# julius-speech/julius

Hardware: NVIDIA H100
Metric: frames/sec (xRT) 20k-word triphone decode (higher is better)
Workload: dtype f32

## Files before the change

### julius_b200/csrc/common.cuh

```cuda
#pragma once
#include <cuda_runtime.h>
#include <cstdint>
#include <cstdio>
#include <cstring>
#include <string>
#include <atomic>
#include <vector>
#include "julius_b200.h"

namespace jb200 {

void set_error(const char *fmt, ...);
extern std::atomic<int64_t> g_launches;

static constexpr int ADDLOG_TABLE_N = 500000;
void build_addlog_table(std::vector<float> &tbl);
__device__ __forceinline__ float addlog_step_exact(float y, float x, const float *__restrict__ tbl) {
  if (x > y) { float t = x; x = y; y = t; }
  float tmp = __fsub_rn(x, y);
  if (tmp < __double2float_ru(JB200_LOG_ADDMIN)) return y;
  unsigned int idx = (unsigned int)__dadd_rn(__dmul_rn((double)(-tmp), 33333.3333), 0.5);
  return __fadd_rn(y, __ldg(tbl + idx));
}

struct SpliceSeg { int row0, frame0, carry0, n_carry, n_win; };
struct SpliceMap {
  const SpliceSeg *seg = nullptr;
  int nseg = 0;
  const float *carry = nullptr;
};
__device__ __forceinline__ const float *splice_frame(const SpliceSeg &s, int k, const float *in, const float *carry, int fl) {
  return (k < s.n_carry) ? carry + (size_t)(s.carry0 + k) * fl : in + (size_t)(s.frame0 + k - s.n_carry) * fl;
}

#define JB_CUDA(expr)                                                              \
  do {                                                                             \
    cudaError_t _e = (expr);                                                       \
    if (_e != cudaSuccess) {                                                       \
      jb200::set_error("%s failed: %s (%s:%d)", #expr, cudaGetErrorString(_e), __FILE__, __LINE__); \
      return JB200_ERR_CUDA;                                                       \
    }                                                                              \
  } while (0)

#define JB_RC(expr)                                                                \
  do {                                                                             \
    const int _rc = (expr);                                                        \
    if (_rc != JB200_OK) return _rc;                                               \
  } while (0)

#define JB_LAUNCH_CHECK()                                                          \
  do {                                                                             \
    jb200::g_launches.fetch_add(1, std::memory_order_relaxed);                     \
    cudaError_t _e = cudaGetLastError();                                           \
    if (_e != cudaSuccess) {                                                       \
      jb200::set_error("kernel launch failed: %s (%s:%d)", cudaGetErrorString(_e), __FILE__, __LINE__); \
      return JB200_ERR_CUDA;                                                       \
    }                                                                              \
  } while (0)

__device__ __forceinline__ uint32_t smem_u32(const void *p) {
  return static_cast<uint32_t>(__cvta_generic_to_shared(p));
}
__device__ __forceinline__ void mbar_init(uint64_t *bar, uint32_t count) {
  asm volatile("mbarrier.init.shared::cta.b64 [%0], %1;" ::"r"(smem_u32(bar)), "r"(count));
}
__device__ __forceinline__ void mbar_fence_init() {
  asm volatile("fence.mbarrier_init.release.cluster;" ::: "memory");
}
__device__ __forceinline__ void mbar_expect_tx(uint64_t *bar, uint32_t bytes) {
  asm volatile("mbarrier.arrive.expect_tx.shared::cta.b64 _, [%0], %1;" ::"r"(smem_u32(bar)), "r"(bytes) : "memory");
}
__device__ __forceinline__ void mbar_wait(uint64_t *bar, uint32_t parity) {
  asm volatile(
      "{\n\t"
      ".reg .pred p;\n\t"
      "WAIT_LOOP:\n\t"
      "mbarrier.try_wait.parity.shared::cta.b64 p, [%0], %1;\n\t"
      "@p bra DONE;\n\t"
      "bra WAIT_LOOP;\n\t"
      "DONE:\n\t"
      "}" ::"r"(smem_u32(bar)), "r"(parity) : "memory");
}
__device__ __forceinline__ void bulk_g2s(void *dst_smem, const void *src_gmem, uint32_t bytes, uint64_t *bar) {
  asm volatile(
      "cp.async.bulk.shared::cluster.global.mbarrier::complete_tx::bytes [%0], [%1], %2, [%3];" ::"r"(smem_u32(dst_smem)),
      "l"(src_gmem), "r"(bytes), "r"(smem_u32(bar))
      : "memory");
}

}
```

### julius_b200/csrc/gmm.cu

```cuda
#include "common.cuh"
#include <cmath>
#include <vector>

namespace jb200 {

static constexpr int GMM_THREADS = 128;
static constexpr int GMM_FPT = 2;
static constexpr int GMM_TILE_STATES = 4;
static constexpr int GMM_TILE_GAUSS = 64;
static constexpr int GMM_NMAX = 16;

__host__ __device__ constexpr int gmm_stride(int D) { return ((2 * D + 2) + 3) & ~3; }

struct GmmTile { int s0, ns, g0, ng; };

__host__ __device__ constexpr int rec_mean(int d) { return 4 * (d >> 1) + (d & 1); }
__host__ __device__ constexpr int rec_ivar(int d) { return 4 * (d >> 1) + 2 + (d & 1); }
__host__ __device__ constexpr int rec_gconst(int D) { return (D & 1) ? 4 * (D >> 1) + 1 : 2 * D; }
__host__ __device__ constexpr int rec_lnw(int D) { return (D & 1) ? 4 * (D >> 1) + 3 : 2 * D + 1; }

__device__ __forceinline__ unsigned long long pack2(float lo, float hi) {
  return ((unsigned long long)__float_as_uint(hi) << 32) | __float_as_uint(lo);
}
__device__ __forceinline__ float lo2(unsigned long long v) { return __uint_as_float((unsigned)(v & 0xffffffffu)); }
__device__ __forceinline__ float hi2(unsigned long long v) { return __uint_as_float((unsigned)(v >> 32)); }
__device__ __forceinline__ unsigned long long fma2(unsigned long long a, unsigned long long b, unsigned long long c) {
  return pack2(__fmaf_rn(lo2(a), lo2(b), lo2(c)), __fmaf_rn(hi2(a), hi2(b), hi2(c)));
}

__device__ __forceinline__ float finish_exact(float lp) {
  if (lp <= JB200_LOG_ZERO || lp == 0.0f) return JB200_LOG_ZERO;
  return (float)((double)lp * JB200_INV_LOG_TEN);
}

__device__ __forceinline__ int cache_push_dev(float *cs, int *ci, int gprune_num, int id, float score, int len) {
  if (len == 0) { cs[0] = score; ci[0] = id; return 1; }
  if (cs[len - 1] >= score) {
    if (len < gprune_num) { cs[len] = score; ci[len] = id; len++; }
    return len;
  }
  int insertp;
  if (cs[0] < score) insertp = 0;
  else {
    int left = 0, right = len - 1;
    while (left < right) { int mid = (left + right) / 2; if (cs[mid] > score) left = mid + 1; else right = mid; }
    insertp = left;
  }
  int last = (len < gprune_num) ? len : len - 1;
  for (int k = last; k > insertp; k--) { cs[k] = cs[k - 1]; ci[k] = ci[k - 1]; }
  cs[insertp] = score; ci[insertp] = id;
  if (len < gprune_num) len++;
  return len;
}

template <int D, bool EXACT, bool PRUNE>
__global__ void __launch_bounds__(GMM_THREADS)
gmm_score_kernel(const float *__restrict__ pk, const GmmTile *__restrict__ tiles, int tiles_per_chunk, int n_tiles,
                 const float *__restrict__ feats, float *__restrict__ rows, int T, int row_stride,
                 const float *__restrict__ tbl, int gprune_num,
                 const int *__restrict__ seg_off, const int *__restrict__ seg_start, int n_seg) {
  constexpr int STRIDE = gmm_stride(D);
  constexpr int NQ = STRIDE / 4;
  __shared__ __align__(128) float buf[2][GMM_TILE_GAUSS * STRIDE];
  __shared__ __align__(8) uint64_t full[2];

  const int tid = threadIdx.x;
  const int f0 = blockIdx.x * (GMM_THREADS * GMM_FPT) + tid;
  const int tile_begin = blockIdx.y * tiles_per_chunk;
  const int tile_end = min(n_tiles, tile_begin + tiles_per_chunk);
  if (tile_begin >= tile_end) return;

  if (tid == 0) { mbar_init(&full[0], 1); mbar_init(&full[1], 1); mbar_fence_init(); }
  __syncthreads();
  if (tid == 0) {
    GmmTile t0 = tiles[tile_begin];
    uint32_t bytes = (uint32_t)t0.ng * STRIDE * 4u;
    mbar_expect_tx(&full[0], bytes);
    bulk_g2s(buf[0], pk + (size_t)t0.g0 * STRIDE, bytes, &full[0]);
  }

  float v[GMM_FPT][D];
  unsigned long long v2[GMM_FPT][NQ];
  int fr[GMM_FPT];
#pragma unroll
  for (int k = 0; k < GMM_FPT; k++) {
    const int fl = f0 + k * GMM_THREADS;
    int fp = min(fl, T - 1);
    if (seg_off != nullptr) {
      int lo = 0, hi = n_seg;
      while (hi - lo > 1) { const int mid = (lo + hi) >> 1; if (__ldg(seg_off + mid) <= fp) lo = mid; else hi = mid; }
      fp = __ldg(seg_start + lo) + (fp - __ldg(seg_off + lo));
    }
    fr[k] = (fl < T) ? fp : -1;
    const float *src = feats + (size_t)fp * D;
#pragma unroll
    for (int d = 0; d < D; d++) v[k][d] = __ldg(src + d);
#pragma unroll
    for (int q = 0; q < NQ; q++) v2[k][q] = pack2((2 * q < D) ? v[k][2 * q < D ? 2 * q : 0] : 0.0f, (2 * q + 1 < D) ? v[k][2 * q + 1 < D ? 2 * q + 1 : 0] : 0.0f);
  }
  const unsigned long long NEG1 = pack2(-1.0f, -1.0f), ZERO2 = pack2(0.0f, 0.0f);

  for (int ti = tile_begin; ti < tile_end; ti++) {
    const int b = (ti - tile_begin) & 1;
    const uint32_t parity = ((ti - tile_begin) >> 1) & 1;
    if (tid == 0 && ti + 1 < tile_end) {
      GmmTile tn = tiles[ti + 1];
      uint32_t bytes = (uint32_t)tn.ng * STRIDE * 4u;
      mbar_expect_tx(&full[b ^ 1], bytes);
      bulk_g2s(buf[b ^ 1], pk + (size_t)tn.g0 * STRIDE, bytes, &full[b ^ 1]);
    }
    const GmmTile tl = tiles[ti];
    mbar_wait(&full[b], parity);
    const float *pb = buf[b];

    int grel = 0;
    for (int si = 0; si < tl.ns; si++) {
      const int *mixcnt = reinterpret_cast<const int *>(tiles + n_tiles);
      const int nm = mixcnt[tl.s0 + si];
      float res[GMM_FPT];
      if (!PRUNE) {
        float y[GMM_FPT], ssum[GMM_FPT];
#pragma unroll
        for (int k = 0; k < GMM_FPT; k++) { y[k] = JB200_LOG_ZERO; ssum[k] = 0.0f; }
        for (int m = nm - 1; m >= 0; m--) {
          const float4 *p = reinterpret_cast<const float4 *>(pb + (size_t)(grel + m) * STRIDE);
          const float gconst = pb[(size_t)(grel + m) * STRIDE + rec_gconst(D)];
          const float lnw = pb[(size_t)(grel + m) * STRIDE + rec_lnw(D)];
          float acc[GMM_FPT];
          unsigned long long acc2[GMM_FPT];
#pragma unroll
          for (int k = 0; k < GMM_FPT; k++) { acc[k] = gconst; acc2[k] = pack2(gconst, 0.0f); }
#pragma unroll
          for (int q = 0; q < NQ; q++) {
            const int d0 = 2 * q, d1 = 2 * q + 1;
            if (d0 < D) {
              const ulonglong2 w = reinterpret_cast<const ulonglong2 *>(p)[q];
#pragma unroll
              for (int k = 0; k < GMM_FPT; k++) {
                const unsigned long long x2 = fma2(w.x, NEG1, v2[k][q]);
                if (EXACT) {
                  const unsigned long long t2 = fma2(fma2(x2, x2, ZERO2), w.y, ZERO2);
                  acc[k] = __fadd_rn(acc[k], lo2(t2));
                  if (d1 < D) acc[k] = __fadd_rn(acc[k], hi2(t2));
                } else {
                  const unsigned long long xi = fma2(x2, w.y, ZERO2);
                  if (d1 < D) acc2[k] = fma2(xi, x2, acc2[k]);
                  else acc[k] = fmaf(lo2(xi), lo2(x2), 0.0f);
                }
              }
            }
          }
          if (!EXACT) {
#pragma unroll
            for (int k = 0; k < GMM_FPT; k++) acc[k] = ((D & 1) ? acc[k] : 0.0f) + lo2(acc2[k]) + hi2(acc2[k]);
          }
          const bool invalid = (gconst != gconst);
#pragma unroll
          for (int k = 0; k < GMM_FPT; k++) {
            float sc = invalid ? JB200_LOG_ZERO : acc[k] * -0.5f;
            if (EXACT) {
              sc = __fadd_rn(sc, lnw);
              y[k] = addlog_step_exact(y[k], sc, tbl);
            } else {
              sc += lnw;
              if (sc > y[k]) { ssum[k] = ssum[k] * __expf(y[k] - sc) + 1.0f; y[k] = sc; }
              else ssum[k] += __expf(sc - y[k]);
            }
          }
        }
#pragma unroll
        for (int k = 0; k < GMM_FPT; k++) {
          if (EXACT) res[k] = finish_exact(y[k]);
          else {
            float lp = y[k] + __logf(ssum[k]);
            res[k] = (nm == 0 || lp <= JB200_LOG_ZERO) ? JB200_LOG_ZERO : lp * (float)JB200_INV_LOG_TEN;
          }
        }
      } else {
#pragma unroll
        for (int k = 0; k < GMM_FPT; k++) {
          float cs[GMM_NMAX]; int ci[GMM_NMAX];
          int num = 0; float thres = JB200_LOG_ZERO;
          for (int m = 0; m < nm; m++) {
            const float *rec = pb + (size_t)(grel + m) * STRIDE;
            const float gconst = rec[rec_gconst(D)];
            float acc = gconst;
#pragma unroll
            for (int d = 0; d < D; d++) {
              float x = __fsub_rn(v[k][d], rec[rec_mean(d)]);
              acc = __fadd_rn(acc, __fmul_rn(__fmul_rn(x, x), rec[rec_ivar(d)]));
            }
            float sc = (gconst != gconst) ? JB200_LOG_ZERO : acc * -0.5f;
            if (num >= gprune_num && sc <= thres) continue;
            num = cache_push_dev(cs, ci, gprune_num, m, sc, num);
            thres = cs[num - 1];
          }
          float y = JB200_LOG_ZERO, ssum = 0.0f;
          for (int i = num - 1; i >= 0; i--) {
            float sc = __fadd_rn(cs[i], pb[(size_t)(grel + ci[i]) * STRIDE + rec_lnw(D)]);
            if (EXACT) y = addlog_step_exact(y, sc, tbl);
            else { if (sc > y) { ssum = ssum * __expf(y - sc) + 1.0f; y = sc; } else ssum += __expf(sc - y); }
          }
          if (EXACT) res[k] = finish_exact(y);
          else { float lp = y + __logf(ssum); res[k] = (num == 0 || lp <= JB200_LOG_ZERO) ? JB200_LOG_ZERO : lp * (float)JB200_INV_LOG_TEN; }
        }
      }
#pragma unroll
      for (int k = 0; k < GMM_FPT; k++)
        if (fr[k] >= 0) rows[(size_t)fr[k] * row_stride + tl.s0 + si] = res[k];
      grel += nm;
    }
    __syncthreads();
  }
}

__global__ void __launch_bounds__(256)
cdset_kernel(float *__restrict__ rows, int T, int row_stride, int S, int C,
             const int *__restrict__ cd_off, const int *__restrict__ cd_states, int method, int maxn) {
  const int c = blockIdx.x * blockDim.x + threadIdx.x;
  const int t = blockIdx.y;
  if (c >= C || t >= T) return;
  const float *st = rows + (size_t)t * row_stride;
  const int b0 = cd_off[c], n_in = cd_off[c + 1] - b0;
  float out;
  if (method == JB200_IWCD_AVG) {
    float sum = 0.0f; int j = 0;
    for (int i = 0; i < n_in; i++) { float p = st[cd_states[b0 + i]]; if (p > JB200_LOG_ZERO) { sum = __fadd_rn(sum, p); j++; } }
    out = __fdiv_rn(sum, (float)j);
  } else if (method == JB200_IWCD_MAX) {
    float mx = JB200_LOG_ZERO;
    for (int i = 0; i < n_in; i++) { float p = st[cd_states[b0 + i]]; if (mx < p) mx = p; }
    out = mx;
  } else {
    float mp[GMM_NMAX + 1]; int n = 0;
    for (int i = 0; i < n_in; i++) {
      float prob = st[cd_states[b0 + i]];
      if (prob <= JB200_LOG_ZERO) continue;
      if (n == 0 || prob <= mp[n - 1]) {
        if (n == maxn) continue;
        mp[n] = prob; n++;
      } else {
        for (int k = 0; k < n; k++) {
          if (prob > mp[k]) {
            int cnt = n - k - ((n == maxn) ? 1 : 0);
            for (int q = k + cnt; q > k; q--) mp[q] = mp[q - 1];
            mp[k] = prob;
            break;
          }
        }
        if (n < maxn) n++;
      }
    }
    float prob = 0.0f;
    for (int i = 0; i < n; i++) prob = __fadd_rn(prob, mp[i]);
    out = __fdiv_rn(prob, (float)n);
  }
  rows[(size_t)t * row_stride + S + c] = out;
}

__global__ void gauss_frame_kernel(const float *__restrict__ pk, int stride, int D, int G,
                                   const float *__restrict__ feat, float *__restrict__ out) {
  int g = blockIdx.x * blockDim.x + threadIdx.x;
  if (g >= G) return;
  const float *rec = pk + (size_t)g * stride;
  float gconst = rec[rec_gconst(D)];
  float acc = gconst;
  for (int d = 0; d < D; d++) {
    float x = __fsub_rn(feat[d], rec[rec_mean(d)]);
    acc = __fadd_rn(acc, __fmul_rn(__fmul_rn(x, x), rec[rec_ivar(d)]));
  }
  out[g] = (gconst != gconst) ? JB200_LOG_ZERO : acc * -0.5f;
}

}

using namespace jb200;

struct jb200_gmm {
  int device = 0, mode = 0;
  int S = 0, D = 0, G = 0, C = 0, max_mix = 0, stride = 0, row_stride = 0;
  int gprune_method = 0, gprune_num = 0, iwcd_method = 0, iwcd_nbest = 0;
  int n_tiles = 0;
  float *d_pk = nullptr;
  GmmTile *d_tiles = nullptr;
  int *d_cd_off = nullptr, *d_cd_states = nullptr;
  float *d_tbl = nullptr;
  cudaStream_t stream = nullptr;
  float *d_feats = nullptr, *d_rows = nullptr; size_t cap_frames = 0;
  int sm_count = 132;
};

namespace jb200 {
int gmm_device(const jb200_gmm *h) { return h->device; }
cudaStream_t gmm_stream(const jb200_gmm *h) { return h->stream; }
int gmm_dim(const jb200_gmm *h) { return h->D; }
int gmm_cd_device(const jb200_gmm *h, const int **cd_off, const int **cd_states, int *method, int *nbest) {
  *cd_off = h->d_cd_off; *cd_states = h->d_cd_states; *method = h->iwcd_method; *nbest = h->iwcd_nbest;
  return 0;
}
}

extern "C" void jb200_gmm_destroy(jb200_gmm *h) {
  if (!h) return;
  cudaSetDevice(h->device);
  cudaFree(h->d_pk); cudaFree(h->d_tiles); cudaFree(h->d_cd_off); cudaFree(h->d_cd_states); cudaFree(h->d_tbl);
  cudaFree(h->d_feats); cudaFree(h->d_rows);
  if (h->stream) cudaStreamDestroy(h->stream);
  delete h;
}

static int gmm_build(jb200_gmm *h, const jb200_gmm_desc *d, const std::vector<int> &mixcnt) {
  JB_CUDA(cudaStreamCreateWithFlags(&h->stream, cudaStreamNonBlocking));

  std::vector<float> pk((size_t)h->G * h->stride, 0.0f);
  for (int g = 0; g < h->G; g++) {
    float *rec = &pk[(size_t)g * h->stride];
    for (int k = 0; k < h->D; k++) { rec[rec_mean(k)] = d->mean[(size_t)g * h->D + k]; rec[rec_ivar(k)] = d->ivar[(size_t)g * h->D + k]; }
    rec[rec_gconst(h->D)] = d->valid[g] ? d->gconst[g] : NAN;
    rec[rec_lnw(h->D)] = d->lnweight[g];
  }
  std::vector<GmmTile> tiles;
  for (int s = 0; s < h->S;) {
    GmmTile t{s, 0, (h->G > 0) ? d->state_off[s] : 0, 0};
    while (s < h->S && t.ns < GMM_TILE_STATES && t.ng + mixcnt[s] <= GMM_TILE_GAUSS) { t.ng += mixcnt[s]; t.ns++; s++; }
    if (t.ng > 0) tiles.push_back(t);
    else if (t.ns == 0) s++;
  }
  h->n_tiles = (int)tiles.size();
  size_t tile_bytes = tiles.size() * sizeof(GmmTile) + mixcnt.size() * sizeof(int);
  std::vector<char> tb(tile_bytes);
  memcpy(tb.data(), tiles.data(), tiles.size() * sizeof(GmmTile));
  memcpy(tb.data() + tiles.size() * sizeof(GmmTile), mixcnt.data(), mixcnt.size() * sizeof(int));

  JB_CUDA(cudaMalloc(&h->d_pk, pk.size() * sizeof(float) + 16));
  if (!pk.empty()) JB_CUDA(cudaMemcpy(h->d_pk, pk.data(), pk.size() * sizeof(float), cudaMemcpyHostToDevice));
  JB_CUDA(cudaMalloc(&h->d_tiles, tile_bytes + 16));
  JB_CUDA(cudaMemcpy(h->d_tiles, tb.data(), tile_bytes, cudaMemcpyHostToDevice));
  if (h->C > 0) {
    JB_CUDA(cudaMalloc(&h->d_cd_off, sizeof(int) * (h->C + 1)));
    JB_CUDA(cudaMemcpy(h->d_cd_off, d->cd_off, sizeof(int) * (h->C + 1), cudaMemcpyHostToDevice));
    JB_CUDA(cudaMalloc(&h->d_cd_states, sizeof(int) * (d->n_cdset_states + 1)));
    JB_CUDA(cudaMemcpy(h->d_cd_states, d->cd_states, sizeof(int) * d->n_cdset_states, cudaMemcpyHostToDevice));
  }
  std::vector<float> tbl;
  build_addlog_table(tbl);
  JB_CUDA(cudaMalloc(&h->d_tbl, tbl.size() * sizeof(float)));
  JB_CUDA(cudaMemcpy(h->d_tbl, tbl.data(), tbl.size() * sizeof(float), cudaMemcpyHostToDevice));
  return JB200_OK;
}

extern "C" int jb200_gmm_create(const jb200_gmm_desc *d, int device, int mode, jb200_gmm **out) {
  if (!d || !out) { set_error("jb200_gmm_create: null argument"); return JB200_ERR_ARG; }
  if (d->gprune_method != JB200_GPRUNE_NONE && (d->gprune_num < 1 || d->gprune_num > GMM_NMAX)) {
    set_error("-tmix %d outside supported range 1..%d", d->gprune_num, GMM_NMAX); return JB200_ERR_UNSUPPORTED;
  }
  if (d->iwcd_method == JB200_IWCD_NBEST && d->iwcd_nbest > GMM_NMAX) { set_error("-iwcd1 best %d too large", d->iwcd_nbest); return JB200_ERR_UNSUPPORTED; }
  std::vector<int> mixcnt(d->n_states);
  for (int s = 0; s < d->n_states; s++) {
    mixcnt[s] = (d->n_gauss > 0) ? d->state_off[s + 1] - d->state_off[s] : 0;
    if (mixcnt[s] > GMM_TILE_GAUSS) { set_error("state %d has %d mixtures (max %d)", s, mixcnt[s], GMM_TILE_GAUSS); return JB200_ERR_UNSUPPORTED; }
  }
  int ndev = 0;
  if (cudaGetDeviceCount(&ndev) != cudaSuccess || ndev <= 0) { set_error("no CUDA device (libjb200 has no CPU fallback)"); return JB200_ERR_NODEVICE; }
// ... 135 lines not shown
```

### julius_b200/csrc/beam.cu

```cuda
#include "common.cuh"
#include "heap_pipe.cuh"
#include <vector>
#include <algorithm>

struct jb200_gmm;
struct jb200_dnn;
namespace jb200 {
int dnn_fix_context(jb200_dnn *h);
int dnn_forward_device(jb200_dnn *h, const float *d_in, int T, float *d_rows, int row_stride, cudaStream_t st, const SpliceMap &sm);
int gmm_device(const jb200_gmm *h);
int gmm_dim(const jb200_gmm *h);
int gmm_launch_states(jb200_gmm *h, const float *d_feats, int T, float *d_rows, int row_stride, cudaStream_t st,
                      const int *seg_off, const int *seg_start, int n_seg);
int gmm_cd_device(const jb200_gmm *h, const int **cd_off, const int **cd_states, int *method, int *nbest);

static constexpr int BEAM_THREADS = 256;
static constexpr int NWARP = BEAM_THREADS / 32;
static constexpr int SEQ_LOCAL_BITS = 18;
static constexpr unsigned SEQ_LOCAL = 1u << SEQ_LOCAL_BITS;
static constexpr int CD_NMAX = 16;
static constexpr int MAX_WORDS = 150;

struct __align__(16) NodeRec { float self_a, next_a; int arc_off, arc_n; int stend, next; int scid, out; };
struct __align__(8) Tok { float score; int node; int tre; int cword; float lscore; int tre_wid; };
// ... 334 lines not shown
      const float xv = hval(pr.x), yv = hval(pr.y), sv = hval(s);
      const bool right = hcmp<MAXHEAP>(xv, yv);
      const unsigned long long c = right ? pr.y : pr.x;
      const float cv = hval(c);
      const bool stop = hstop<MAXHEAP>(sv, cv) || (MAXHEAP && cv < lose_below);
      const unsigned long long put = stop ? s : c;
      store_slot(slot, put);
      if (slot == 1) outs[my_x + 1] = put;
      if (stop) act = false;
      else { slot = 2 * cur + (right ? 1 : 0); cur = min(slot, cap); }
    }
    __syncwarp();
    if (--wait <= 0) {
      if (next_x >= extract) { if (!__any_sync(FULL, act)) break; }
      else {
        const int ms = n - next_x;
        const int ln = next_x & (NL - 1);
        bool blocks = act && ((int)lane == ln);
        if (!(MAXHEAP && hval(nxt) < lose_below)) {
          const int dh = 31 - __clz(max(slot, 1)), dms = 31 - __clz(ms);
          blocks = blocks || (act && dms >= dh && (ms >> (dms - dh)) == slot);
        }
        if (!__any_sync(FULL, blocks)) {
          if ((int)lane == ln) {
            s = load_slot(ms);
            store_slot(ms, sent);
            my_x = next_x; act = true; slot = 1; cur = 1;
          }
          next_x++; wait = 2;
          nxt = load_slot(n - next_x);
        } else stalls++;
      }
    }
    __syncwarp();
    ticks++;
  }
  ticks_out = ticks; stalls_out = stalls;
}

struct SlotClear {
  const Tok *tok; int n; SlotView slots;
  __device__ __forceinline__ void run(int first, int stride) const {
    for (int i = first; i < n; i += stride) {
      const int node = tok[i].node;
      slots.reset(node);
    }
  }
};

template <bool MAXHEAP>
__device__ __forceinline__ void heap_pad_sentinels(unsigned long long *A, const int n, const int maxt) {
  const unsigned long long sent = MAXHEAP ? 0xff800000ull : 0x7f800000ull;
  const int hi = min(2 * n + 1, maxt + 1);
  for (int i = n + 1 + (int)threadIdx.x; i <= hi; i += BEAM_THREADS) A[i] = sent;
  if (threadIdx.x < 2) A[maxt + 2 + threadIdx.x] = sent;
}

extern __shared__ __align__(16) unsigned char beam_smem[];
struct CutAreas {
  unsigned long long *heap;
  int *offs;
  unsigned long long *gq; int gqn;
  unsigned long long *gtail; int gtn;
  __device__ __forceinline__ unsigned long long *outv() const { return reinterpret_cast<unsigned long long *>(offs); }
};
__device__ __forceinline__ CutAreas cut_areas(const BeamParams &p) {
  unsigned long long *const smem_q = reinterpret_cast<unsigned long long *>(beam_smem);
  CutAreas a;
  a.heap = p.heap_g ? p.heap_g + (size_t)blockIdx.x * (p.maxt + 4) : smem_q;
  a.offs = reinterpret_cast<int *>(smem_q + (p.heap_g ? p.qcap : p.maxt + 4));
  a.gq = p.heap_g ? smem_q : nullptr;
  a.gqn = p.heap_g ? p.qcap : 0;
  a.gtail = p.heap_g ? reinterpret_cast<unsigned long long *>(a.offs + 2 * (p.beam + 2)) : nullptr;
  a.gtn = p.heap_g ? p.beam + 1 : 0;
  return a;
}

template <bool MAXHEAP>
__device__ void heap_extract_fast(const CutAreas &ca, const int n, const int extract, const float lose_below, const int maxt,
                                  unsigned long long *stats, const SlotClear *idle_work = nullptr) {
  unsigned long long *const A = ca.heap, *const outv = ca.outv(), *const gcache = ca.gq;
  HeapCache hc{nullptr, 0, nullptr, 0, 0};
  if (!__isShared(A) && n + 8 <= ca.gqn) {
    const int lmaxt = (ca.gqn - 4) & ~1;
    for (int i = threadIdx.x; i <= n; i += BEAM_THREADS) gcache[i] = A[i];
    heap_pad_sentinels<MAXHEAP>(gcache, n, lmaxt);
    __syncthreads();
    if (threadIdx.x >= 32 && idle_work) idle_work->run((int)threadIdx.x - 32, BEAM_THREADS - 32);
    if (threadIdx.x < 32) {
      unsigned ticks, stalls;
      heap_extract_pipe_warp6<MAXHEAP>(gcache, n, extract, lose_below, outv, lmaxt, threadIdx.x, ticks, stalls);
      if (threadIdx.x == 0) {
        atomicAdd(stats + CUT_REPLAY_TICKS, (unsigned long long)ticks); atomicAdd(stats + CUT_REPLAY_EXTRACTS, (unsigned long long)extract);
        atomicAdd(stats + CUT_HELD_BACK, (unsigned long long)stalls); atomicAdd(stats + CUT_GLOBAL_WHOLE, 1ull);
      }
    }
    __syncthreads();
    for (int i = 1 + threadIdx.x; i <= n; i += BEAM_THREADS) A[i] = gcache[i];
    __syncthreads();
    return;
  }
  if (!__isShared(A)) {
    hc.top = gcache; hc.cs = min(ca.gqn, maxt + 4) & ~1;
    for (int i = threadIdx.x; i < hc.cs; i += BEAM_THREADS) gcache[i] = A[i];
    if (ca.gtn >= extract) {
      hc.tail = ca.gtail; hc.tail_first = n - extract + 1; hc.tail_n = extract;
      for (int i = threadIdx.x; i < extract; i += BEAM_THREADS) ca.gtail[i] = A[hc.tail_first + i];
    }
    __syncthreads();
  }
  if (threadIdx.x >= 32 && idle_work) idle_work->run((int)threadIdx.x - 32, BEAM_THREADS - 32);
  if (threadIdx.x < 32) {
    unsigned ticks, stalls;
    if (!__isShared(A)) heap_extract_pipe_global<MAXHEAP>(A, n, extract, lose_below, outv, maxt, hc, ticks, stalls);
    else heap_extract_pipe_warp6<MAXHEAP>(A, n, extract, lose_below, outv, maxt, threadIdx.x, ticks, stalls);
    if (threadIdx.x == 0) {
      atomicAdd(stats + CUT_REPLAY_TICKS, (unsigned long long)ticks); atomicAdd(stats + CUT_REPLAY_EXTRACTS, (unsigned long long)extract);
      atomicAdd(stats + CUT_HELD_BACK, (unsigned long long)stalls);
      if (!__isShared(A)) atomicAdd(stats + CUT_GLOBAL_TOP_TAIL, 1ull);
    }
  }
  __syncthreads();
}

__device__ __forceinline__ int closed_subtree_size(const int c, const int n, const int H) {
  const int dc = 31 - __clz(c);
  if (dc > H) return 0;
  const int sh = H - dc;
  const int first = c << sh, width = 1 << sh;
  return (width - 1) + max(0, min(n - first + 1, width));
}

constexpr int RELOC_WINDOW = 3;
__device__ __forceinline__ void reloc_window_load(const unsigned long long *keys, const int nc, const int base, const int skip, const int lane,
                                                  unsigned (&pre)[(RELOC_WINDOW + 1) / 2]) {
#pragma unroll
  for (int c = 0; c < RELOC_WINDOW; c++) {
    const int idx = base + 32 * c + lane;
    const unsigned p = (idx < nc && idx != skip) ? 0xffffu - (unsigned)((keys[idx] >> 16) & 0xffffu) : 0xffffu;
    if (c & 1) pre[c >> 1] |= p << 16; else pre[c >> 1] = p;
  }
}
__device__ __forceinline__ int reloc_window_first(const unsigned (&pre)[(RELOC_WINDOW + 1) / 2], const int lo, const int hi, const int from, const int lane) {
  int f = -1;
#pragma unroll
  for (int c = RELOC_WINDOW - 1; c >= 0; c--) {
    const int p = (int)((pre[c >> 1] >> (16 * (c & 1))) & 0xffffu);
    const unsigned b = __ballot_sync(0xffffffffu, p >= lo && p < hi && 32 * c + lane >= from);
    if (b) f = 32 * c + __ffs(b) - 1;
  }
  return f;
}

__device__ __forceinline__ int closed_relocate(unsigned long long *keys, const int nc, const int n, const int need, unsigned *flags, unsigned *multi,
                                            unsigned *pay, const int lane) {
  constexpr unsigned FULL = 0xffffffffu;
  const int H = 31 - __clz(n);
  const int tail0 = n - need + 1, fwords = (need + 31) >> 5;
  for (int w = fwords - 1; w >= 0; w--) {
    unsigned bits = flags[w];
    while (bits) {
      const int b = 31 - __clz(bits);
      const int m = tail0 + w * 32 + b;
      const int k = n - m + 1;
      if (m <= n && m >= 2 && k <= need) {
        const int dm = 31 - __clz(m);
        const bool is_multi = (multi[(m - tail0) >> 5] >> ((m - tail0) & 31)) & 1u;
        int j = 0, a = 1, lo = 0, hi = n, occ = -1;
        bool gone = false;
        for (int base = k - 1; base < nc && occ < 0 && !gone; base += 32 * RELOC_WINDOW) {
          unsigned pre[(RELOC_WINDOW + 1) / 2];
          reloc_window_load(keys, nc, base, -1, lane, pre);
          int from = 0;
          while (true) {
            const int f = reloc_window_first(pre, lo, hi, from, lane);
            if (f < 0) break;
            if (j == dm) { occ = base + f; break; }
            if (!is_multi && (int)(pay[(unsigned)keys[base + f] & 0xffffu] >> 16) == m) { gone = true; break; }
            j++;
            const int nxt = m >> (dm - j);
            const int lsz = closed_subtree_size(2 * a, n, H);
            if (nxt == 2 * a) { lo = lo + 1; hi = lo + lsz; } else { lo = lo + 1 + lsz; }
            a = nxt;
            from = f + 1;
          }
        }
        if (occ >= k) {
          __syncwarp();
          const unsigned long long ekey = keys[occ];
          const unsigned esc = (unsigned)(ekey >> 32);
          const int msz = m - 1;
          int x = 1; lo = 0; hi = n;
          bool stop = (2 * x > msz);
          for (int base = k; base < nc && !stop; base += 32 * RELOC_WINDOW) {
            unsigned pre[(RELOC_WINDOW + 1) / 2];
            reloc_window_load(keys, nc, base, occ, lane, pre);
            int from = 0;
            while (!stop) {
              const int f = reloc_window_first(pre, lo, hi, from, lane);
              if (f < 0) break;
              const unsigned long long fk = keys[base + f];
              const unsigned osc = (unsigned)(fk >> 32);
              const int opre = 0xffff - (int)((fk >> 16) & 0xffffu);
              if (opre == lo) return 0;
              if (esc >= osc) { stop = true; break; }
              const int lsz = closed_subtree_size(2 * x, n, H);
              if (opre < lo + 1 + lsz) { x = 2 * x; lo = lo + 1; hi = lo + lsz; }
              else { x = 2 * x + 1; lo = lo + 1 + lsz; }
              if (2 * x > msz) { stop = true; break; }
              from = f + 1;
            }
          }
          const unsigned long long nkey = (ekey & 0xffffffff0000ffffull) | ((unsigned long long)(0xffffu - (unsigned)lo) << 16);
          int cnt = 0;
          {
            const int wb = max(k, occ - 16), we = wb + 31;
            const bool lo_ok = (wb == k) || ((unsigned)(keys[wb] >> 32) > esc);
            const bool hi_ok = (we >= nc) || ((unsigned)(keys[we] >> 32) < esc);
            if (lo_ok && hi_ok) {
              const int idx = wb + lane;
              const bool gt = (idx < nc) && idx != occ && keys[idx] > nkey;
              cnt = (wb - k) + __popc(__ballot_sync(FULL, gt));
            } else {
              for (int base = k; base < nc; base += 32) {
                const int idx = base + lane;
                const bool gt = (idx < nc) && idx != occ && keys[idx] > nkey;
                const unsigned mask = __ballot_sync(FULL, gt);
                cnt += __popc(mask);
                const bool le = (idx < nc) && idx != occ && !gt;
                if (__any_sync(FULL, le)) break;
              }
            }
          }
          const int ins = k + cnt;
          if (ins < occ) {
            for (int top = occ; top > ins; top -= 32) {
              const int idx = top - lane;
              unsigned long long v = 0ull;
              if (idx > ins) v = keys[idx - 1];
              __syncwarp();
              if (idx > ins) keys[idx] = v;
              __syncwarp();
            }
          } else if (ins > occ) {
            for (int bot = occ; bot < ins; bot += 32) {
              const int idx = bot + lane;
              unsigned long long v = 0ull;
              if (idx < ins) v = keys[idx + 1];
              __syncwarp();
              if (idx < ins) keys[idx] = v;
              __syncwarp();
            }
          }
          if (lane == 0) {
            keys[ins] = nkey;
            unsigned *pp = pay + ((unsigned)nkey & 0xffffu);
            *pp = ((unsigned)x << 16) | (*pp & 0xffffu);
            if (x >= tail0 && x < m) { flags[(x - tail0) >> 5] |= 1u << ((x - tail0) & 31); multi[(x - tail0) >> 5] |= 1u << ((x - tail0) & 31); }
          }
          __syncwarp();
        }
      }
      bits = flags[w] & ((b == 0) ? 0u : ((1u << b) - 1u));
    }
  }
  return 1;
}

constexpr int SORT_TILE = 128;
__device__ __forceinline__ void sort_cx(unsigned long long &a, unsigned long long &b, const bool desc) {
  if (desc ? (a < b) : (a > b)) { const unsigned long long t = a; a = b; b = t; }
}
__device__ __forceinline__ void sort_tile_pass(unsigned long long *keys, const int nc, const int np, const int k_lo, const int k_hi) {
  const int lane = threadIdx.x & 31;
  for (int i0 = (threadIdx.x >> 5) * SORT_TILE + lane; i0 - lane < np; i0 += (BEAM_THREADS >> 5) * SORT_TILE) {
    unsigned long long v[4];
#pragma unroll
    for (int r = 0; r < 4; r++) v[r] = (i0 + 32 * r < nc) ? keys[i0 + 32 * r] : 0ull;
    for (int k = k_lo; k <= k_hi; k <<= 1) {
      if (k >= 128) { sort_cx(v[0], v[2], (i0 & k) == 0); sort_cx(v[1], v[3], (i0 & k) == 0); }
      if (k >= 64) { sort_cx(v[0], v[1], (i0 & k) == 0); sort_cx(v[2], v[3], ((i0 + 64) & k) == 0); }
      for (int j = min(k >> 1, 16); j > 0; j >>= 1) {
        const bool low = ((lane & j) == 0);
#pragma unroll
        for (int r = 0; r < 4; r++) {
          const unsigned long long o = __shfl_xor_sync(0xffffffffu, v[r], j);
          const bool keep_max = (low == (((i0 + 32 * r) & k) == 0));
          if (keep_max == (o > v[r])) v[r] = o;
        }
      }
    }
#pragma unroll
    for (int r = 0; r < 4; r++) if (i0 + 32 * r < np) keys[i0 + 32 * r] = v[r];
  }
  __syncthreads();
}

__device__ int heap_select_closed(unsigned long long *heap, const int n, const int need, const float lose_below, const int maxt,
                                  unsigned long long *keys, const int key_cap, unsigned *pay, const int pay_cap,
                                  int *ordn, int *s_scratch ) {
  const int tid = threadIdx.x;
  int relocated = 0;
  if (n >= 65536 || maxt >= 65536 || !(lose_below > -INFINITY)) return 0;
  const int tail0 = n - need + 1, fwords = (need + 31) >> 5;
  unsigned *const flags = pay + pay_cap - fwords, *const multi = pay + pay_cap - 2 * fwords;
  const bool have_flags = (2 * fwords < pay_cap);
  if (tid == 0) { s_scratch[0] = 0; s_scratch[1] = 0; }
  if (have_flags) for (int i = tid; i < 2 * fwords; i += BEAM_THREADS) multi[i] = 0u;
  __syncthreads();
  const int H = 31 - __clz(n);
  const int cap = min(min(key_cap, have_flags ? pay_cap - 2 * fwords : pay_cap), 65535);
  for (int h0 = 1; h0 <= n; h0 += BEAM_THREADS) {
    const int h = h0 + tid;
    unsigned long long e = 0ull;
    bool is_c = false;
    if (h <= n) { e = heap[h]; is_c = (hval(e) >= lose_below); }
    const unsigned m = __ballot_sync(0xffffffffu, is_c);
    int base = 0;
    if ((tid & 31) == 0 && m) base = atomicAdd(&s_scratch[0], __popc(m));
    base = __shfl_sync(0xffffffffu, base, 0);
    if (is_c) {
      const int ci = base + __popc(m & ((1u << (tid & 31)) - 1u));
      if (ci < cap) {
        keys[ci] = ((unsigned long long)fkey(hval(e)) << 32) | (unsigned)ci;
        pay[ci] = ((unsigned)h << 16) | (unsigned)(e >> 32);
      }
    }
  }
  __syncthreads();
  const int nc = s_scratch[0];
  int np = 1; while (np < nc) np <<= 1;
  if (nc > cap || np > key_cap || nc < need) return 0;
  const bool can_relocate = have_flags;
  for (int ci = tid; ci < nc; ci += BEAM_THREADS) {
    const int h = (int)(pay[ci] >> 16), d = 31 - __clz(h);
    int pre = d;
    for (int b = d - 1; b >= 0; b--) {
      if ((h >> b) & 1) {
        const int sh = H - (d - b), width = 1 << sh;
        pre += (width - 1) + max(0, min(n - ((((h >> b) ^ 1)) << sh) + 1, width));
      }
    }
    keys[ci] |= (unsigned long long)(0xffffu - (unsigned)pre) << 16;
  }
  __syncthreads();
  sort_tile_pass(keys, nc, np, 2, min(np, SORT_TILE));
  for (int k = 2 * SORT_TILE; k <= np; k <<= 1) {
    for (int j = k >> 1; j >= SORT_TILE; j >>= 1) {
      for (int i = tid; i < (np >> 1); i += BEAM_THREADS) {
        const int a = ((i & ~(j - 1)) << 1) | (i & (j - 1)), b = a | j;
        const unsigned long long ka = keys[a], kb = keys[b];
        const bool desc = ((a & k) == 0);
        if (desc ? (ka < kb) : (ka > kb)) { keys[a] = kb; keys[b] = ka; }
      }
      __syncthreads();
    }
    sort_tile_pass(keys, np, np, k, k);
  }
  const unsigned theta = (unsigned)(keys[need - 1] >> 32);
  for (int i = tid; i < nc; i += BEAM_THREADS) {
    const unsigned long long ki = keys[i];
    const unsigned sk = (unsigned)(ki >> 32);
    if (sk < theta) continue;
    const int slot = (int)(pay[(unsigned)ki & 0xffffu] >> 16);
    if (slot < tail0) continue;
    const bool tied = (i > 0 && (unsigned)(keys[i - 1] >> 32) == sk) || (i + 1 < nc && (unsigned)(keys[i + 1] >> 32) == sk);
    int last = i;
    if (tied) { int g = 0; while (last + 1 < nc && (unsigned)(keys[last + 1] >> 32) == sk && g < 8) { last++; g++; } if (g == 8) last = nc; }
    const int kstep = n - slot + 1, d = 31 - __clz(slot);
    if (last + 1 < kstep + d) continue;
    if (have_flags) atomicOr(flags + ((slot - tail0) >> 5), 1u << ((slot - tail0) & 31));
    if (tied) s_scratch[1] = 1;
  }
  __syncthreads();
  if (s_scratch[1]) {
    if (!can_relocate) return 0;
    if (tid < 32) { const int ok = closed_relocate(keys, nc, n, need, flags, multi, pay, tid); if (tid == 0) s_scratch[1] = ok ? 2 : 1; }
    __syncthreads();
    if (s_scratch[1] != 2) return 0;
    relocated = 1;
  }
  for (int k = tid; k < need; k += BEAM_THREADS) ordn[k] = (int)(pay[(unsigned)keys[need - 1 - k] & 0xffffu] & 0xffffu);
  return 1 + relocated;
}


__device__ int trace_backptr(const jb200_atom *atoms, int a, int *w) {
  int n = 0;
  w[n++] = atoms[a].wid;
  while (atoms[a].begintime > 0) {
    a = atoms[a].last;
    if (a < 0 || n >= MAX_WORDS) break;
    w[n++] = atoms[a].wid;
  }
  for (int i = 0; i < n / 2; i++) { const int x = w[i]; w[i] = w[n - 1 - i]; w[n - 1 - i] = x; }
  return n;
}

__device__ void interim_best(const BeamParams &p, const int u, const jb200_atom *araw, const int lo, const int hi, const int frame) {
  UttState *st = p.state + u;
  int best = -1; float mx = JB200_LOG_ZERO;
  for (int a = hi - 1; a >= lo; a--) if (mx < araw[a].backscore) { mx = araw[a].backscore; best = a; }
  st->interim_frame = frame - 1;
  if (best < 0) { st->interim_nwords = 0; st->interim_score = JB200_LOG_ZERO; return; }
  st->interim_nwords = trace_backptr(araw, best, p.interim_words + (size_t)u * MAX_WORDS); st->interim_score = mx;
}

#define PROF_MARK(k) do { if (tid == 0) { long long _n = clock64(); s_prof[k] += _n - s_tprev; s_tprev = _n; } } while (0)

__device__ __forceinline__ void beam_cut(const BeamParams &p, const CutAreas &ca, const int n, const unsigned &s_maxkey,
                                         const Tok *tn, const SlotView &slots, int *ordn, long long *s_prof, long long &s_tprev) {
  __shared__ unsigned s_losekey;
  __shared__ int s_cf[2];
  const int tid = threadIdx.x;
  const int need = p.beam, maxt = p.maxt;
  unsigned long long *const heap = ca.heap, *const outv = ca.outv();
  const SlotClear sc{tn, n, slots};
  if (need < n - need) {
    constexpr int NB = 1024;
    int *hist = ca.offs;
    const int nb = min(NB, 2 * (p.beam + 2));
    for (int i = tid; i < nb; i += BEAM_THREADS) hist[i] = 0;
    __syncthreads();
    const unsigned maxkey = s_maxkey;
    const int e = (int)((((maxkey & 0x80000000u) ? (maxkey & 0x7fffffffu) : ~maxkey) >> 23) & 0xffu) - 127;
    const int sh = max(0, min(24, 22 - e));
    for (int r = tid; r < n; r += BEAM_THREADS) {
      const unsigned key = fkey(hval(heap[r + 1]));
      const unsigned bin = min((unsigned)(nb - 1), (maxkey - key) >> sh);
      atomicAdd(&hist[bin], 1);
    }
    __syncthreads();
    if (tid < 32) {
      int cum = 0, found = -1;
      for (int b0 = 0; b0 < nb && found < 0; b0 += 32) {
        const int v = (b0 + tid < nb) ? hist[b0 + tid] : 0;
        int x = v;
        for (int o = 1; o < 32; o <<= 1) { int y = __shfl_up_sync(0xffffffffu, x, o); if (tid >= o) x += y; }
        const unsigned hit = __ballot_sync(0xffffffffu, cum + x >= need);
        if (hit) found = b0 + __ffs(hit) - 1;
        cum += __shfl_sync(0xffffffffu, x, 31);
      }
      if (tid == 0) {
        unsigned lk = 0u;
        if (found >= 0 && found < nb - 1) {
          const unsigned long long drop = (unsigned long long)(found + 1) << sh;
          lk = (drop < maxkey) ? maxkey - (unsigned)drop : 0u;
        }
        s_losekey = lk;
      }
    }
    __syncthreads();
    const unsigned lk = s_losekey;
    const float lose_below = (lk == 0u) ? -INFINITY : __uint_as_float((lk & 0x80000000u) ? (lk & 0x7fffffffu) : ~lk);
    heap_build<true>(heap, n); PROF_MARK(7);
    sc.run(tid, BEAM_THREADS);
    const int closed = heap_select_closed(heap, n, need, lose_below, maxt, ca.gq ? ca.gq : heap + n + 1, ca.gq ? p.sort_cap : maxt + 3 - n,
                                          reinterpret_cast<unsigned *>(ca.offs), 2 * (p.beam + 2), ordn, s_cf);
    if (tid == 0) {
      atomicAdd(p.cut_counters + CUT_UPWARD, 1ull);
      if (closed) atomicAdd(p.cut_counters + CUT_CLOSED, 1ull);
      if (closed == 2) atomicAdd(p.cut_counters + CUT_RELOCATED, 1ull);
    }
    if (!closed) {
      heap_pad_sentinels<true>(heap, n, maxt);
      __syncthreads();
      heap_extract_fast<true>(ca, n, need, lose_below, maxt, p.cut_counters);
      for (int k = tid; k < need; k += BEAM_THREADS) ordn[k] = (int)(outv[need - 1 - k] >> 32);
    }
  } else {
    heap_pad_sentinels<false>(heap, n, maxt);
    heap_build<false>(heap, n); PROF_MARK(7);
    heap_extract_fast<false>(ca, n, n - need, -INFINITY, maxt, p.cut_counters, &sc);
    for (int k = tid; k < need; k += BEAM_THREADS) ordn[k] = (int)(heap[k + 1] >> 32);
  }
}

template <bool GRAMMAR>
__device__ __forceinline__ void finalize_utt(const BeamParams &p, const int u, const int tid, const int T, jb200_atom *araw, int *newidx,
                                             const int *group0, jb200_utt_result *res, int *words,
                                             int &s_natoms, int &s_overflow, int &s_found, long long &s_outbase,
                                             long long *s_prof, long long &s_tprev) {
  const int natoms = s_natoms;
  for (int a = tid; a < natoms; a += BEAM_THREADS) {
    const jb200_atom me = araw[a];
    const int lo = group0[me.endtime], hi = group0[me.endtime + 1];
    int rank = 0;
    for (int b = lo; b < hi; b++) rank += (araw[b].wid < me.wid) ? 1 : 0;
    newidx[a] = lo + rank;
  }
  if (tid == 0) {
    if (p.atoms_in_place) s_outbase = p.atom_off[u];
    else {
      unsigned long long base = atomicAdd(p.atom_counter, (unsigned long long)natoms);
      if ((long long)(base + natoms) > p.atoms_out_cap) { s_overflow = 1; s_outbase = -1; }
      else s_outbase = (long long)base;
    }
  }
  __syncthreads();
  const long long ob = s_outbase;
  const bool can_write = (ob >= 0);
  const int kept = can_write ? natoms : 0;
  for (int a = tid; a < kept; a += BEAM_THREADS) {
    jb200_atom me = araw[a];
    me.last = (me.last < 0) ? -1 : newidx[me.last];
    p.atoms_out[ob + newidx[a]] = me;
    if ((GRAMMAR || me.wid == p.tail_silwid) && me.backscore > JB200_LOG_ZERO) atomicMax(&s_found, me.endtime);
  }
  __threadfence_block();
  __syncthreads();

  if (tid == 0) {
    int status = 0, nw = 0; float score = 0.0f;
    const int last_time = s_found;
    if (kept == 0 || last_time < 0) status = -1;
    else {
      const jb200_atom *const atoms = p.atoms_out + ob;
      const int lo = group0[last_time], hi = group0[last_time + 1];
      int best = -1;
      if constexpr (GRAMMAR) {
        float maxscore = JB200_LOG_ZERO;
        for (int b = lo; b < hi; b++) {
          const jb200_atom x = atoms[b];
          if (maxscore < x.backscore) { maxscore = x.backscore; best = b; }
        }
      } else {
        for (int b = lo; b < hi; b++) {
          const jb200_atom x = atoms[b];
          if (x.wid == p.tail_silwid && x.backscore > JB200_LOG_ZERO) { best = b; break; }
        }
      }
      if (best < 0) status = -1;
// ... 2023 lines not shown
```

Measured before the change: 1.212 million.

## Interleave two states' mixture walks and split addlog table lookup for ILP

In the non-pruned GMM path, two HMM states are processed together, with their Gaussian loops interleaved so independent dependency chains overlap. The exact addlog step is split into an issue phase that starts the table load and a finish phase that applies it one iteration later, hiding load latency. This raises register pressure and adds predicated wasted work when the two states have different mixture counts.

```diff
diff --git a/julius_b200/csrc/common.cuh b/julius_b200/csrc/common.cuh
--- a/julius_b200/csrc/common.cuh
+++ b/julius_b200/csrc/common.cuh
@@ -15,12 +15,18 @@
 
 static constexpr int ADDLOG_TABLE_N = 500000;
 void build_addlog_table(std::vector<float> &tbl);
+struct AddlogStep { float y, t; bool add; };
+__device__ __forceinline__ AddlogStep addlog_issue(float y, float x, bool on, const float *__restrict__ tbl) {
+  const bool swap = on && x > y;
+  const float hi = swap ? x : y, lo = swap ? y : x;
+  const float tmp = __fsub_rn(lo, hi);
+  const bool add = on && !(tmp < __double2float_ru(JB200_LOG_ADDMIN));
+  const unsigned int idx = (unsigned int)__dadd_rn(__dmul_rn((double)(-tmp), 33333.3333), 0.5);
+  return AddlogStep{hi, add ? __ldg(tbl + idx) : 0.0f, add};
+}
+__device__ __forceinline__ float addlog_finish(const AddlogStep &s) { return s.add ? __fadd_rn(s.y, s.t) : s.y; }
 __device__ __forceinline__ float addlog_step_exact(float y, float x, const float *__restrict__ tbl) {
-  if (x > y) { float t = x; x = y; y = t; }
-  float tmp = __fsub_rn(x, y);
-  if (tmp < __double2float_ru(JB200_LOG_ADDMIN)) return y;
-  unsigned int idx = (unsigned int)__dadd_rn(__dmul_rn((double)(-tmp), 33333.3333), 0.5);
-  return __fadd_rn(y, __ldg(tbl + idx));
+  return addlog_finish(addlog_issue(y, x, true, tbl));
 }
 
 struct SpliceSeg { int row0, frame0, carry0, n_carry, n_win; };
diff --git a/julius_b200/csrc/gmm.cu b/julius_b200/csrc/gmm.cu
--- a/julius_b200/csrc/gmm.cu
+++ b/julius_b200/csrc/gmm.cu
@@ -51,6 +51,93 @@
   cs[insertp] = score; ci[insertp] = id;
   if (len < gprune_num) len++;
   return len;
+}
+
+template <int D, bool EXACT, int NS>
+__device__ __forceinline__ void gmm_walk(const float *pb, int g0, const int *nm, const unsigned long long (&v2)[GMM_FPT][gmm_stride(D) / 4],
+                                         const float *__restrict__ tbl, float *__restrict__ rows, const int (&fr)[GMM_FPT],
+                                         int row_stride, int s0) {
+  constexpr int STRIDE = gmm_stride(D);
+  constexpr int NQ = STRIDE / 4;
+  const unsigned long long NEG1 = pack2(-1.0f, -1.0f), ZERO2 = pack2(0.0f, 0.0f);
+  int n[NS], gs[NS], nmax = 0, nmin = GMM_TILE_GAUSS;
+#pragma unroll
+  for (int j = 0; j < NS; j++) {
+    n[j] = nm[j]; gs[j] = (j == 0) ? g0 : gs[j - 1] + n[j - 1];
+    nmax = max(nmax, n[j]); nmin = min(nmin, n[j]);
+  }
+  AddlogStep st[NS][GMM_FPT];
+  float y[NS][GMM_FPT], ssum[NS][GMM_FPT];
+#pragma unroll
+  for (int j = 0; j < NS; j++)
+#pragma unroll
+    for (int k = 0; k < GMM_FPT; k++) { st[j][k] = AddlogStep{JB200_LOG_ZERO, 0.0f, false}; y[j][k] = JB200_LOG_ZERO; ssum[j][k] = 0.0f; }
+  auto gauss = [&](int j, int m, bool on) {
+    const int g = on ? gs[j] + m : 0;
+    const float4 *p = reinterpret_cast<const float4 *>(pb + (size_t)g * STRIDE);
+    const float gconst = pb[(size_t)g * STRIDE + rec_gconst(D)];
+    const float lnw = pb[(size_t)g * STRIDE + rec_lnw(D)];
+    float acc[GMM_FPT];
+    unsigned long long acc2[GMM_FPT];
+#pragma unroll
+    for (int k = 0; k < GMM_FPT; k++) { acc[k] = gconst; acc2[k] = pack2(gconst, 0.0f); }
+#pragma unroll
+    for (int q = 0; q < NQ; q++) {
+      const int d0 = 2 * q, d1 = 2 * q + 1;
+      if (d0 < D) {
+        const ulonglong2 w = reinterpret_cast<const ulonglong2 *>(p)[q];
+#pragma unroll
+        for (int k = 0; k < GMM_FPT; k++) {
+          const unsigned long long x2 = fma2(w.x, NEG1, v2[k][q]);
+          if (EXACT) {
+            const unsigned long long t2 = fma2(fma2(x2, x2, ZERO2), w.y, ZERO2);
+            acc[k] = __fadd_rn(acc[k], lo2(t2));
+            if (d1 < D) acc[k] = __fadd_rn(acc[k], hi2(t2));
+          } else {
+            const unsigned long long xi = fma2(x2, w.y, ZERO2);
+            if (d1 < D) acc2[k] = fma2(xi, x2, acc2[k]);
+            else acc[k] = fmaf(lo2(xi), lo2(x2), 0.0f);
+          }
+        }
+      }
+    }
+    if (!EXACT) {
+#pragma unroll
+      for (int k = 0; k < GMM_FPT; k++) acc[k] = ((D & 1) ? acc[k] : 0.0f) + lo2(acc2[k]) + hi2(acc2[k]);
+    }
+    const bool invalid = (gconst != gconst);
+#pragma unroll
+    for (int k = 0; k < GMM_FPT; k++) {
+      float sc = invalid ? JB200_LOG_ZERO : acc[k] * -0.5f;
+      if (EXACT) {
+        sc = __fadd_rn(sc, lnw);
+        st[j][k] = addlog_issue(addlog_finish(st[j][k]), sc, on, tbl);
+      } else {
+        sc += lnw;
+        const bool up = sc > y[j][k];
+        const float s1 = up ? ssum[j][k] * __expf(y[j][k] - sc) + 1.0f : ssum[j][k] + __expf(sc - y[j][k]);
+        if (on) { ssum[j][k] = s1; y[j][k] = up ? sc : y[j][k]; }
+      }
+    }
+  };
+  for (int m = nmax - 1; m >= nmin; m--)
+#pragma unroll
+    for (int j = 0; j < NS; j++) gauss(j, m, m < n[j]);
+  for (int m = nmin - 1; m >= 0; m--)
+#pragma unroll
+    for (int j = 0; j < NS; j++) gauss(j, m, true);
+#pragma unroll
+  for (int j = 0; j < NS; j++)
+#pragma unroll
+    for (int k = 0; k < GMM_FPT; k++) {
+      float res;
+      if (EXACT) res = finish_exact(addlog_finish(st[j][k]));
+      else {
+        const float lp = y[j][k] + __logf(ssum[j][k]);
+        res = (n[j] == 0 || lp <= JB200_LOG_ZERO) ? JB200_LOG_ZERO : lp * (float)JB200_INV_LOG_TEN;
+      }
+      if (fr[k] >= 0) rows[(size_t)fr[k] * row_stride + s0 + j] = res;
+    }
 }
 
 template <int D, bool EXACT, bool PRUNE>
@@ -98,7 +185,6 @@
 #pragma unroll
     for (int q = 0; q < NQ; q++) v2[k][q] = pack2((2 * q < D) ? v[k][2 * q < D ? 2 * q : 0] : 0.0f, (2 * q + 1 < D) ? v[k][2 * q + 1 < D ? 2 * q + 1 : 0] : 0.0f);
   }
-  const unsigned long long NEG1 = pack2(-1.0f, -1.0f), ZERO2 = pack2(0.0f, 0.0f);
 
   for (int ti = tile_begin; ti < tile_end; ti++) {
     const int b = (ti - tile_begin) & 1;
@@ -113,70 +199,19 @@
     mbar_wait(&full[b], parity);
     const float *pb = buf[b];
 
+    const int *mixcnt = reinterpret_cast<const int *>(tiles + n_tiles);
     int grel = 0;
-    for (int si = 0; si < tl.ns; si++) {
-      const int *mixcnt = reinterpret_cast<const int *>(tiles + n_tiles);
-      const int nm = mixcnt[tl.s0 + si];
-      float res[GMM_FPT];
-      if (!PRUNE) {
-        float y[GMM_FPT], ssum[GMM_FPT];
-#pragma unroll
-        for (int k = 0; k < GMM_FPT; k++) { y[k] = JB200_LOG_ZERO; ssum[k] = 0.0f; }
-        for (int m = nm - 1; m >= 0; m--) {
-          const float4 *p = reinterpret_cast<const float4 *>(pb + (size_t)(grel + m) * STRIDE);
-          const float gconst = pb[(size_t)(grel + m) * STRIDE + rec_gconst(D)];
-          const float lnw = pb[(size_t)(grel + m) * STRIDE + rec_lnw(D)];
-          float acc[GMM_FPT];
-          unsigned long long acc2[GMM_FPT];
-#pragma unroll
-          for (int k = 0; k < GMM_FPT; k++) { acc[k] = gconst; acc2[k] = pack2(gconst, 0.0f); }
-#pragma unroll
-          for (int q = 0; q < NQ; q++) {
-            const int d0 = 2 * q, d1 = 2 * q + 1;
-            if (d0 < D) {
-              const ulonglong2 w = reinterpret_cast<const ulonglong2 *>(p)[q];
-#pragma unroll
-              for (int k = 0; k < GMM_FPT; k++) {
-                const unsigned long long x2 = fma2(w.x, NEG1, v2[k][q]);
-                if (EXACT) {
-                  const unsigned long long t2 = fma2(fma2(x2, x2, ZERO2), w.y, ZERO2);
-                  acc[k] = __fadd_rn(acc[k], lo2(t2));
-                  if (d1 < D) acc[k] = __fadd_rn(acc[k], hi2(t2));
-                } else {
-                  const unsigned long long xi = fma2(x2, w.y, ZERO2);
-                  if (d1 < D) acc2[k] = fma2(xi, x2, acc2[k]);
-                  else acc[k] = fmaf(lo2(xi), lo2(x2), 0.0f);
-                }
-              }
-            }
-          }
-          if (!EXACT) {
-#pragma unroll
-            for (int k = 0; k < GMM_FPT; k++) acc[k] = ((D & 1) ? acc[k] : 0.0f) + lo2(acc2[k]) + hi2(acc2[k]);
-          }
-          const bool invalid = (gconst != gconst);
-#pragma unroll
-          for (int k = 0; k < GMM_FPT; k++) {
-            float sc = invalid ? JB200_LOG_ZERO : acc[k] * -0.5f;
-            if (EXACT) {
-              sc = __fadd_rn(sc, lnw);
-              y[k] = addlog_step_exact(y[k], sc, tbl);
-            } else {
-              sc += lnw;
-              if (sc > y[k]) { ssum[k] = ssum[k] * __expf(y[k] - sc) + 1.0f; y[k] = sc; }
-              else ssum[k] += __expf(sc - y[k]);
-            }
-          }
-        }
-#pragma unroll
-        for (int k = 0; k < GMM_FPT; k++) {
-          if (EXACT) res[k] = finish_exact(y[k]);
-          else {
-            float lp = y[k] + __logf(ssum[k]);
-            res[k] = (nm == 0 || lp <= JB200_LOG_ZERO) ? JB200_LOG_ZERO : lp * (float)JB200_INV_LOG_TEN;
-          }
-        }
-      } else {
+    if (!PRUNE) {
+      int si = 0;
+      for (; si + 1 < tl.ns; si += 2) {
+        gmm_walk<D, EXACT, 2>(pb, grel, mixcnt + tl.s0 + si, v2, tbl, rows, fr, row_stride, tl.s0 + si);
+        grel += mixcnt[tl.s0 + si] + mixcnt[tl.s0 + si + 1];
+      }
+      if (si < tl.ns) gmm_walk<D, EXACT, 1>(pb, grel, mixcnt + tl.s0 + si, v2, tbl, rows, fr, row_stride, tl.s0 + si);
+    } else {
+      for (int si = 0; si < tl.ns; si++) {
+        const int nm = mixcnt[tl.s0 + si];
+        float res[GMM_FPT];
 #pragma unroll
         for (int k = 0; k < GMM_FPT; k++) {
           float cs[GMM_NMAX]; int ci[GMM_NMAX];
@@ -204,11 +239,11 @@
           if (EXACT) res[k] = finish_exact(y);
           else { float lp = y + __logf(ssum); res[k] = (num == 0 || lp <= JB200_LOG_ZERO) ? JB200_LOG_ZERO : lp * (float)JB200_INV_LOG_TEN; }
         }
+#pragma unroll
+        for (int k = 0; k < GMM_FPT; k++)
+          if (fr[k] >= 0) rows[(size_t)fr[k] * row_stride + tl.s0 + si] = res[k];
+        grel += nm;
       }
-#pragma unroll
-      for (int k = 0; k < GMM_FPT; k++)
-        if (fr[k] >= 0) rows[(size_t)fr[k] * row_stride + tl.s0 + si] = res[k];
-      grel += nm;
     }
     __syncthreads();
   }
```

New measurement: 1.239 million, median of 6. 1.02x the previous value.

## Index candidate ranks in heap spare bits to shortcut closed relocation walks

Applied to the files above, without the earlier changes.

Stores each candidate's sorted-key rank in the unused top 16 bits of its heap entry, indexed by preorder position. Once a relocation subtree narrows to 32 or fewer positions, the walk switches from window scans to a warp-wide min-reduction over those stored ranks. The ranks are kept current as keys shift and the relocated key moves, with a marker for positions holding more than one candidate. This adds an index-building pass and extra writes, lowers the key cap by one, and must clear the heap's high bits when relocation fails, so correctness depends on those bits being otherwise unused.

```diff
diff --git a/julius_b200/csrc/beam.cu b/julius_b200/csrc/beam.cu
--- a/julius_b200/csrc/beam.cu
+++ b/julius_b200/csrc/beam.cu
@@ -510,8 +510,18 @@
   return f;
 }
 
-__device__ __forceinline__ int closed_relocate(unsigned long long *keys, const int nc, const int n, const int need, unsigned *flags, unsigned *multi,
-                                            unsigned *pay, const int lane) {
+constexpr unsigned RANK_MULTI = 0xffffu;
+__device__ __forceinline__ unsigned short *rank_at(unsigned long long *heap, const int pos) {
+  return reinterpret_cast<unsigned short *>(heap + pos + 1) + 3;
+}
+__device__ __forceinline__ void rank_note(unsigned long long *heap, const int pos, const int idx) {
+  unsigned short *const r = rank_at(heap, pos);
+  if (*r != RANK_MULTI) *r = (unsigned short)(idx + 1);
+}
+constexpr int RELOC_INDEX_SPAN = 32;
+
+__device__ __forceinline__ int closed_relocate(unsigned long long *keys, unsigned long long *heap, const int nc, const int n, const int need,
+                                            unsigned *flags, unsigned *multi, unsigned *pay, const int lane) {
   constexpr unsigned FULL = 0xffffffffu;
   const int H = 31 - __clz(n);
   const int tail0 = n - need + 1, fwords = (need + 31) >> 5;
@@ -541,6 +551,26 @@
             if (nxt == 2 * a) { lo = lo + 1; hi = lo + lsz; } else { lo = lo + 1 + lsz; }
             a = nxt;
             from = f + 1;
+            if (hi - lo <= RELOC_INDEX_SPAN) {
+              const unsigned v = (lo + lane < hi) ? *rank_at(heap, lo + lane) : 0u;
+              if (!__any_sync(FULL, v == RANK_MULTI)) {
+                const int r = (int)v - 1, pos = lo + lane;
+                int fa = base + f + 1;
+                for (;;) {
+                  const unsigned mn = __reduce_min_sync(FULL, (pos >= lo && pos < hi && r >= fa) ? (unsigned)r : 0xffffffffu);
+                  if (mn == 0xffffffffu) break;
+                  if (j == dm) { occ = (int)mn; break; }
+                  j++;
+                  const int nx = m >> (dm - j);
+                  const int ls = closed_subtree_size(2 * a, n, H);
+                  if (nx == 2 * a) { lo = lo + 1; hi = lo + ls; } else { lo = lo + 1 + ls; }
+                  a = nx;
+                  fa = (int)mn + 1;
+                }
+                gone = (occ < 0);
+                break;
+              }
+            }
           }
         }
         if (occ >= k) {
@@ -567,6 +597,29 @@
               else { x = 2 * x + 1; lo = lo + 1 + lsz; }
               if (2 * x > msz) { stop = true; break; }
               from = f + 1;
+              if (hi - lo <= RELOC_INDEX_SPAN) {
+                const unsigned v = (lo + lane < hi) ? *rank_at(heap, lo + lane) : 0u;
+                if (!__any_sync(FULL, v == RANK_MULTI)) {
+                  const int r = (int)v - 1, pos = lo + lane;
+                  const unsigned sc = (r >= 0) ? (unsigned)(keys[r] >> 32) : 0u;
+                  int fa = base + f + 1;
+                  for (;;) {
+                    const unsigned mn = __reduce_min_sync(FULL, (pos >= lo && pos < hi && r >= fa && r != occ) ? (unsigned)r : 0xffffffffu);
+                    if (mn == 0xffffffffu) break;
+                    const int l = __ffs(__ballot_sync(FULL, r == (int)mn)) - 1;
+                    const int op = __shfl_sync(FULL, pos, l);
+                    if (op == lo) return 0;
+                    if (esc >= __shfl_sync(FULL, sc, l)) break;
+                    const int ls = closed_subtree_size(2 * x, n, H);
+                    if (op < lo + 1 + ls) { x = 2 * x; lo = lo + 1; hi = lo + ls; }
+                    else { x = 2 * x + 1; lo = lo + 1 + ls; }
+                    if (2 * x > msz) break;
+                    fa = (int)mn + 1;
+                  }
+                  stop = true;
+                  break;
+                }
+              }
             }
           }
           const unsigned long long nkey = (ekey & 0xffffffff0000ffffull) | ((unsigned long long)(0xffffu - (unsigned)lo) << 16);
@@ -597,7 +650,7 @@
               unsigned long long v = 0ull;
               if (idx > ins) v = keys[idx - 1];
               __syncwarp();
-              if (idx > ins) keys[idx] = v;
+              if (idx > ins) { keys[idx] = v; rank_note(heap, 0xffff - (int)((v >> 16) & 0xffffu), idx); }
               __syncwarp();
             }
           } else if (ins > occ) {
@@ -606,7 +659,7 @@
               unsigned long long v = 0ull;
               if (idx < ins) v = keys[idx + 1];
               __syncwarp();
-              if (idx < ins) keys[idx] = v;
+              if (idx < ins) { keys[idx] = v; rank_note(heap, 0xffff - (int)((v >> 16) & 0xffffu), idx); }
               __syncwarp();
             }
           }
@@ -615,6 +668,11 @@
             unsigned *pp = pay + ((unsigned)nkey & 0xffffu);
             *pp = ((unsigned)x << 16) | (*pp & 0xffffu);
             if (x >= tail0 && x < m) { flags[(x - tail0) >> 5] |= 1u << ((x - tail0) & 31); multi[(x - tail0) >> 5] |= 1u << ((x - tail0) & 31); }
+            unsigned short *const eold = rank_at(heap, 0xffff - (int)((ekey >> 16) & 0xffffu));
+            if (*eold != RANK_MULTI) *eold = 0;
+            unsigned short *const xr = rank_at(heap, lo);
+            const unsigned old = *xr;
+            *xr = (old == 0u || (old != RANK_MULTI && (int)old - 1 < k)) ? (unsigned short)(ins + 1) : (unsigned short)RANK_MULTI;
           }
           __syncwarp();
         }
@@ -667,7 +725,7 @@
   if (have_flags) for (int i = tid; i < 2 * fwords; i += BEAM_THREADS) multi[i] = 0u;
   __syncthreads();
   const int H = 31 - __clz(n);
-  const int cap = min(min(key_cap, have_flags ? pay_cap - 2 * fwords : pay_cap), 65535);
+  const int cap = min(min(key_cap, have_flags ? pay_cap - 2 * fwords : pay_cap), 65534);
   for (int h0 = 1; h0 <= n; h0 += BEAM_THREADS) {
     const int h = h0 + tid;
     unsigned long long e = 0ull;
@@ -733,9 +791,14 @@
   __syncthreads();
   if (s_scratch[1]) {
     if (!can_relocate) return 0;
-    if (tid < 32) { const int ok = closed_relocate(keys, nc, n, need, flags, multi, pay, tid); if (tid == 0) s_scratch[1] = ok ? 2 : 1; }
-    __syncthreads();
-    if (s_scratch[1] != 2) return 0;
+    for (int i = tid; i < nc; i += BEAM_THREADS) *rank_at(heap, 0xffff - (int)((keys[i] >> 16) & 0xffffu)) = (unsigned short)(i + 1);
+    __syncthreads();
+    if (tid < 32) { const int ok = closed_relocate(keys, heap, nc, n, need, flags, multi, pay, tid); if (tid == 0) s_scratch[1] = ok ? 2 : 1; }
+    __syncthreads();
+    if (s_scratch[1] != 2) {
+      for (int h = 1 + tid; h <= n; h += BEAM_THREADS) heap[h] &= 0x0000ffffffffffffull;
+      return 0;
+    }
     relocated = 1;
   }
   for (int k = tid; k < need; k += BEAM_THREADS) ordn[k] = (int)(pay[(unsigned)keys[need - 1 - k] & 0xffffu] & 0xffffu);
```

Result: faster. 1.213 million before, 1.228 million after, median of 6 (+1.3%).
